# ShengkaiWu/IoU-aware-single-stage-object-detector

Hardware: AMD Instinct MI355X
Metric: images/sec at 1333x800, IoU-aware RetinaNet R-50-FPN (higher is better)
Workload: dtype fp32; 1 GPU; IoU-aware RetinaNet R-50-FPN fp32, batch 8 per GPU, 3x800x1344 (1333x800 padded to /32), random-init weights, whole inference path incl. NMS, device-to-host copy and bbox2result (the reference's simple_test: per-class arrays on the host; batch i's host part runs under batch i+1's device part, the last one inside the timed region); global_batch=8, parallelism=dp1, dets_per_image=100

## Files before the change

### include/iouaware.h

```cpp
#ifndef IOUAWARE_H
#define IOUAWARE_H

#include <stddef.h>
#include <stdint.h>

#ifdef __cplusplus
extern "C" {
#endif

#define IA_MAX_LEVELS 8
#define IA_MAX_ANCHORS 16
#define IA_MAX_NMS_PRE 4096
#define IA_MAX_CANDIDATES 8192
#define IA_MAX_PER_IMG 1024

#define IA_F32 0
#define IA_BF16 1
#define IA_F16 2
#define IA_F64 3

#define IA_LAYOUT_NCHW 0
#define IA_LAYOUT_NHWC 1

#define IA_CLS_SIGMOID 0
// ... 152 lines not shown
int ia_bn_fold_bwd(const float *dw_folded, const float *db_folded, const float *w, const float *gamma,
                   const float *mean, const float *inv_std, int cout, int K, float *dw,
                   float *dgamma, float *dbeta, void *stream);
int ia_relu_bwd_bias_grad(const float *dy, const float *y, int64_t rows, int n, float *g, float *db,
                          void *workspace, size_t workspace_bytes, void *stream);

int ia_linear_bias_act(const float *A, const float *W, const float *bias, const float *residual,
                       float *D, int64_t rows, int k, int n, int relu, void *workspace,
                       size_t workspace_bytes, void *stream);
int ia_linear_bias_act_bf16(const void *A, const void *W, const float *bias, const void *residual,
                            void *D, int64_t rows, int k, int n, int relu, void *workspace,
                            size_t workspace_bytes, void *stream);
int ia_batched_gemm(const float *A, const float *W, float *D, int batch, int64_t rows, int k, int n,
                    void *workspace, size_t workspace_bytes, void *stream);
int ia_batched_gemm_stream(const float *A, const float *W, float *D, int batch, int64_t rows, int k,
                           int n, void *stream);

size_t ia_im2col3x3_bytes(int B, int H, int W, int C, int stride, int dtype);
int ia_im2col3x3_nhwc(const void *x, void *col, int B, int H, int W, int C, int stride, int dtype,
                      void *stream);
int ia_conv1x1_strided(const void *x, const void *W_kn, const float *bias, const void *residual,
                       void *D, int B, int H, int W, int k, int n, int stride, int relu, int dtype,
                       void *workspace, size_t workspace_bytes, void *stream);
int ia_col2im3x3_nhwc(const void *dcol, void *dx, int B, int H, int W, int C, int stride, int dtype,
                      void *stream);

size_t ia_deform_im2col3x3_bytes(int B, int H, int W, int C, int stride, int pad, int dil);
int ia_deform_im2col3x3_nhwc(const float *x, const float *offset, int64_t offset_pix_stride,
                             const float *mask, int64_t mask_pix_stride, int mask_logits,
                             float *col, int B, int H, int W, int C, int stride, int pad,
                             int dil, int deformable_groups, void *stream);
int ia_deform_col2im3x3_nhwc(const float *dcol, const float *x, const float *offset,
                             int64_t offset_pix_stride, const float *mask,
                             int64_t mask_pix_stride, float *dx, float *d_offset, float *d_mask,
                             int B, int H, int W, int C, int stride, int pad, int dil,
                             int deformable_groups, void *stream);

int ia_gemm_tuning(int mode);

int ia_gemm_table_add(int64_t m, int64_t n, int64_t k, int flags, int batch, int dtype,
                      int solution_index);
int ia_gemm_table_clear(void);
int ia_gemm_table_dump(int64_t *rows7, int capacity);
int ia_gemm_table_stats(int64_t *hits_misses_stale);
int ia_gemm_library_version(void);

// ... 176 lines not shown

int ia_affine_relu_maxpool_nhwc(const float *x, const float *scale, const float *shift, int B, int H,
                                int W, int C, float *out, void *stream);
int ia_affine_relu_maxpool_nhwc_dt(const void *x, int dtype, const float *scale, const float *shift,
                                   int B, int H, int W, int C, void *out, void *stream);

int ia_upsample2x_add_nhwc(float *fine, const float *coarse, int B, int H, int W, int Hc, int Wc,
                           int C, void *stream);
int ia_upsample2x_add_nhwc_dt(void *fine, const void *coarse, int dtype, int B, int H, int W, int Hc,
                              int Wc, int C, void *stream);

int ia_stem_conv7x7s2(const float *x, const float *w_packed, float *y, int B, int H, int W,
                      void *stream);
int ia_stem_conv7x7s2_bf16(const void *x, const void *w_packed, void *y, int B, int H, int W,
                           void *stream);

int ia_conv1x1_stream(const float *x, const float *w, const float *bias, const float *residual,
                      float *y, int64_t rows, int k, int n, int relu, void *stream);
int ia_conv1x1_chain(const float *x, const float *w, const float *bias, const float *residual,
                     const float *w2, const float *bias2, float *y, float *h, int64_t rows, int k,
                     int n, int n2, void *stream);
int ia_conv1x1_wide(const float *x, const float *w, const float *bias, const float *residual,
                    float *y, int64_t rows, int k, int n, int relu, void *stream);

typedef struct ia_conv3x3_desc {
    int32_t num_levels, batch, groups;
    int32_t cin, cout;
    int32_t x_stride, y_stride;
    int32_t H[IA_MAX_LEVELS], W[IA_MAX_LEVELS];
    const void *x[2][IA_MAX_LEVELS];
    void *y[2][IA_MAX_LEVELS];
} ia_conv3x3_desc;
size_t ia_conv3x3_bf16_packed_bytes(int cin, int cout, int groups);
int ia_conv3x3_bf16_pack(const void *w, int cin, int cout, int groups, void *wp, void *stream);
int ia_conv3x3_bf16_levels(const ia_conv3x3_desc *d, const void *wp, const float *bias, int relu, void *stream);

size_t ia_conv3x3_bf16_wgrad_workspace_bytes(const ia_conv3x3_desc *d);
int ia_conv3x3_bf16_wgrad_plan(const ia_conv3x3_desc *d, int32_t *tiles, int32_t *slice_tiles, int32_t *slices);
int ia_conv3x3_bf16_wgrad_levels(const ia_conv3x3_desc *d, float *dw, void *workspace, size_t workspace_bytes,
                                 void *stream);
int ia_conv3x3_bf16_pack_f32(const float *w, int cin, int cout, int groups, int adjoint, void *wp, void *stream);
size_t ia_relu_bwd_bias_grad_bf16_workspace_bytes(int64_t rows, int n);
int ia_relu_bwd_bias_grad_bf16(const void *dy, int64_t dy_stride, const void *y, int64_t y_stride, int64_t rows,
                               int n, void *g, int64_t g_stride, float *db, void *workspace,
                               size_t workspace_bytes, void *stream);

// ... 155 lines not shown
```

### iou-aware-single-stage-object-detector_amd/csrc/build.py

```python
import os
import subprocess
import sys

HERE = os.path.dirname(os.path.abspath(__file__))
SOURCES = ['capi.hip', 'decode.hip', 'select.hip', 'nms.hip', 'loss.hip', 'elementwise.hip', 'assign.hip',
           'softnms.hip', 'preproc.hip', 'wino.hip', 'gemm.hip', 'lazynms.hip', 'headloss.hip', 'gconv.hip',
           'trainops.hip', 'bignms.hip', 'conv3x3_bf16.hip', 'conv3x3_bf16_bwd.hip', 'conv1x1_stream.hip', 'im2col.hip', 'nms64.hip', 'stem.hip',
           'groupnorm.hip', 'pointdecode.hip', 'pointloss.hip', 'gconv_bf16.hip', 'gconv_bwd.hip', 'deform.hip']
HEADERS = ['ia_math.hpp', 'ia_block.hpp', 'ia_internal.hpp', 'ia_loss.hpp', 'ia_headloss.hpp', 'ia_rowmax_dev.hpp', 'ia_gather_dev.hpp', 'ia_nms.hpp', 'ia_conv3.hpp', 'ia_wino.hpp', '../../include/iouaware.h']
OUT = os.path.join(HERE, 'libiouaware_hip.so')
FLAGS = ['--offload-arch=gfx950', '-O3', '-std=c++17', '-fPIC', '-ffp-contract=off',
         '-fhip-fp32-correctly-rounded-divide-sqrt', '-fno-gpu-rdc',
         '-Wall', '-Wno-unused-function']


def _hipcc():
    for c in (os.environ.get('HIPCC'), '/opt/rocm/bin/hipcc', 'hipcc'):
        if c and (os.path.isabs(c) and os.path.exists(c) or not os.path.isabs(c)):
            return c
    return 'hipcc'


def needs_build():
    if not os.path.exists(OUT):
        return True
    t = os.path.getmtime(OUT)
    deps = [os.path.join(HERE, f) for f in SOURCES + HEADERS] + [os.path.abspath(__file__)]
    return any(os.path.getmtime(d) > t for d in deps)


def build(force=False, verbose=False):
    if not force and not needs_build():
# ... 25 lines not shown
```

### iou-aware-single-stage-object-detector_amd/csrc/conv1x1_stream.hip

```cpp
#include <string.h>
#include <mutex>
#include <vector>
#include "ia_internal.hpp"

namespace ia {

typedef __attribute__((ext_vector_type(4))) float f32x4;

struct Conv1Args {
    const float *x, *w, *bias, *res;
    float *y;
    int64_t P;
    int32_t relu, tiles;
    int64_t xs, ws, ys;
};

constexpr int kC1Threads = 512;

template <int K, int N>
__global__ void __launch_bounds__(kC1Threads) __attribute__((amdgpu_waves_per_eu(4, 4))) k_conv1x1_stream(Conv1Args a)
{
    constexpr int NB = N / 16, J = K / 16, LDW = N + 4;
    __shared__ __attribute__((aligned(16))) float s_w[K * LDW];
    __shared__ __attribute__((aligned(16))) float s_bias[N];
    const int tid = threadIdx.x, lane = tid & 63;
    a.x += (size_t)blockIdx.y * a.xs; a.w += (size_t)blockIdx.y * a.ws; a.y += (size_t)blockIdx.y * a.ys;
// ... 117 lines not shown
                const float *wrow = wq + (16 * j + c) * LDW;
                constexpr int WB = NB > 8 ? 8 : NB;
#pragma unroll
                for (int n0 = 0; n0 < NB; n0 += WB) {
                    float wf[WB];
#pragma unroll
                    for (int nb = 0; nb < WB; ++nb) wf[nb] = wrow[16 * (n0 + nb)];
#pragma unroll
                    for (int nb = 0; nb < WB; ++nb)
                        acc[n0 + nb] = __builtin_amdgcn_mfma_f32_16x16x4f32(wf[nb], xb, acc[n0 + nb], 0, 0, 0);
                    if (n0 + WB < NB) __builtin_amdgcn_sched_barrier(0);
                }
                __builtin_amdgcn_sched_barrier(0);
            }
        if (p0 < a.P) {
            float *yr = a.y + p * a.ldn + n0 + 4 * q;
#pragma unroll
            for (int nb = 0; nb < NB; ++nb) {
                f32x4 v = acc[nb];
                if (a.relu) { v.x = v.x > 0.f ? v.x : 0.f; v.y = v.y > 0.f ? v.y : 0.f; v.z = v.z > 0.f ? v.z : 0.f; v.w = v.w > 0.f ? v.w : 0.f; }
                *reinterpret_cast<f32x4 *>(yr + 16 * nb) = v;
            }
        }
    }
}

struct ChainArgs {
    const float *x, *w, *bias, *res;
    const float *w2, *bias2;
    float *y, *h;
    int64_t P;
    int32_t tiles;
};

constexpr int kChainThreads = 1024;

template <int K, int N, int N2>
__global__ void __launch_bounds__(kChainThreads) __attribute__((amdgpu_waves_per_eu(4, 4))) k_conv1x1_chain(ChainArgs a)
{
    constexpr int NB = N / 16, J = K / 16, LDW = N + 4, NB2 = N2 / 16, LDW2 = N2 + 4;
    extern __shared__ __attribute__((aligned(16))) float s_dyn[];
    float *s_w = s_dyn, *s_w2 = s_w + K * LDW, *s_bias = s_w2 + N * LDW2, *s_bias2 = s_bias + N;
    const int tid = threadIdx.x, lane = tid & 63;
    for (int i = tid; i < K * (N / 4); i += kChainThreads) {
        const int k = i / (N / 4), n4 = i - k * (N / 4);
        *reinterpret_cast<float4 *>(s_w + k * LDW + 4 * n4) = *reinterpret_cast<const float4 *>(a.w + (size_t)k * N + 4 * n4);
// ... 186 lines not shown
    if (tiles > 2147483647LL) return IA_E_ARG;
    a.tiles = (int32_t)tiles;
    int64_t wgs = (tiles + 15) / 16;
    if (wgs > 128) wgs = 128;
    const size_t lds = sizeof(float) * (128 * (256 + 4) + 256);
    int dev = 0;
    if (hipGetDevice(&dev) != hipSuccess) return IA_E_ARG;
    {
        static std::mutex mu;
        static std::vector<char> done;
        std::lock_guard<std::mutex> lock(mu);
        if ((size_t)dev >= done.size()) done.resize((size_t)dev + 1, 0);
        if (!done[dev]) {
            hipError_t e = hipFuncSetAttribute(reinterpret_cast<const void *>(&ia::k_conv1x1_wide<128, 256>),
                                               hipFuncAttributeMaxDynamicSharedMemorySize, (int)lds);
            if (e != hipSuccess) return ia::hip_status(e);
            done[dev] = 1;
        }
    }
    hipLaunchKernelGGL((ia::k_conv1x1_wide<128, 256>), dim3((unsigned)wgs, 2), dim3(ia::kWideThreads), lds,
                       (hipStream_t)stream, a);
    return ia::hip_status(hipGetLastError());
}
```

### iou-aware-single-stage-object-detector_amd/csrc/im2col.hip

```cpp
#include "ia_internal.hpp"

namespace ia {

struct Im2colArgs {
    const uint4 *x;
    uint4 *col;
    int32_t B, H, W, Ho, Wo, stride;
    int32_t cv;
    int32_t lanes;
    int64_t runs;
};

__global__ __launch_bounds__(256) void k_im2col3x3(Im2colArgs a)
{
    const int lane = threadIdx.x & 63;
    const int sub = lane / a.lanes, l = lane - sub * a.lanes;
    const int per_wave = 64 / a.lanes;
    const int64_t wave = (int64_t)blockIdx.x * 4 + (threadIdx.x >> 6);
    for (int r = 0; r < 4; ++r) {
        const int64_t run = (wave * 4 + r) * per_wave + sub;
        if (run >= a.runs) return;
        const int64_t pix = run / 9;
        const int tap = (int)(run - pix * 9);
        const int dy = tap / 3, dx = tap - dy * 3;
        const int xo = (int)(pix % a.Wo);
        const int64_t t = pix / a.Wo;
        const int yo = (int)(t % a.Ho);
        const int b = (int)(t / a.Ho);
        const int yi = yo * a.stride + dy - 1, xi = xo * a.stride + dx - 1;
        const bool in = yi >= 0 && yi < a.H && xi >= 0 && xi < a.W;
        const uint4 *src = a.x + (((int64_t)b * a.H + (in ? yi : 0)) * a.W + (in ? xi : 0)) * a.cv;
        uint4 *dst = a.col + run * a.cv;
        for (int c = l; c < a.cv; c += a.lanes) {
            uint4 v = src[c];
            if (!in) v = make_uint4(0, 0, 0, 0);
            dst[c] = v;
        }
    }
}

struct Col2imArgs {
    const float4 *dcol;
    float4 *dx;
    int32_t H, W, Ho, Wo;
    int32_t cv;
    int32_t shift;
};

template <int S>
__global__ __launch_bounds__(256) void k_col2im3x3(Col2imArgs a)
{
    constexpr int NJ = (S + 2) / S;
    const int lane = threadIdx.x & 63;
    const int lanes = 1 << a.shift, sub = lane >> a.shift, l = lane & (lanes - 1);
    const int per_wave = 64 >> a.shift;
    const int xi = ((int)blockIdx.y * 4 + (int)(threadIdx.x >> 6)) * per_wave + sub;
    if (xi >= a.W) return;
    const int row = (int)blockIdx.x;
    const int b = row / a.H, yi = row - b * a.H;
    const int dy0 = (yi + 1) % S, dx0 = (xi + 1) % S;
    int64_t off[NJ * NJ];
    bool ok[NJ * NJ];
#pragma unroll
    for (int j = 0; j < NJ; ++j) {
        const int dy = dy0 + j * S, ny = yi + 1 - dy, yo = ny / S;
        const bool oky = dy < 3 && ny >= 0 && yo < a.Ho;
#pragma unroll
        for (int i = 0; i < NJ; ++i) {
            const int dx = dx0 + i * S, nx = xi + 1 - dx, xo = nx / S;
            const bool in = oky && dx < 3 && nx >= 0 && xo < a.Wo;
            ok[j * NJ + i] = in;
            off[j * NJ + i] = in ? ((((int64_t)b * a.Ho + yo) * a.Wo + xo) * 9 + (dy * 3 + dx)) * a.cv : 0;
        }
    }
    float4 *dst = a.dx + ((int64_t)row * a.W + xi) * a.cv;
    for (int c = l; c < a.cv; c += lanes) {
        float4 v[NJ * NJ];
#pragma unroll
        for (int t = 0; t < NJ * NJ; ++t) v[t] = a.dcol[off[t] + c];
        float4 acc = make_float4(0.0f, 0.0f, 0.0f, 0.0f);
#pragma unroll
        for (int t = 0; t < NJ * NJ; ++t)
            if (ok[t]) { acc.x += v[t].x; acc.y += v[t].y; acc.z += v[t].z; acc.w += v[t].w; }
        dst[c] = acc;
    }
}

}

extern "C" size_t ia_im2col3x3_bytes(int B, int H, int W, int C, int stride, int dtype)
{
    if (B < 1 || H < 1 || W < 1 || C < 1 || stride < 1 || (dtype != IA_F32 && dtype != IA_BF16)) return 0;
    const int64_t Ho = (H - 1) / stride + 1, Wo = (W - 1) / stride + 1;
// ... 2 lines not shown

extern "C" int ia_im2col3x3_nhwc(const void *x, void *col, int B, int H, int W, int C, int stride,
                                 int dtype, void *stream)
{
    if (!x || !col || B < 1 || H < 1 || W < 1 || C < 1 || stride < 1 || stride > 4) return IA_E_ARG;
    if (dtype != IA_F32 && dtype != IA_BF16) return IA_E_ARG;
    const int esz = dtype == IA_F32 ? 4 : 2;
    if ((C * esz) % 16) return IA_E_ARG;
    if (((uintptr_t)x | (uintptr_t)col) & 15) return IA_E_ARG;
    ia::Im2colArgs a;
    a.x = (const uint4 *)x; a.col = (uint4 *)col;
    a.B = B; a.H = H; a.W = W; a.stride = stride;
    a.Ho = (H - 1) / stride + 1; a.Wo = (W - 1) / stride + 1;
    a.cv = C * esz / 16;
    int lanes = 64;
    while (lanes > a.cv) lanes >>= 1;
    a.lanes = lanes < 1 ? 1 : lanes;
    a.runs = (int64_t)B * a.Ho * a.Wo * 9;
    const int64_t per_block = 16LL * (64 / a.lanes);
    const int64_t blocks = (a.runs + per_block - 1) / per_block;
    if (blocks > 2147483647LL) return IA_E_ARG;
    hipLaunchKernelGGL(ia::k_im2col3x3, dim3((unsigned)blocks), dim3(256), 0, (hipStream_t)stream, a);
    return ia::hip_status(hipGetLastError());
}

extern "C" int ia_col2im3x3_nhwc(const void *dcol, void *dx, int B, int H, int W, int C, int stride,
                                 int dtype, void *stream)
{
    if (!dcol || !dx || B < 1 || H < 1 || W < 1 || C < 1 || stride < 1 || stride > 4) return IA_E_ARG;
    if (dtype != IA_F32 || C % 4) return IA_E_ARG;
    if (((uintptr_t)dcol | (uintptr_t)dx) & 15) return IA_E_ARG;
    ia::Col2imArgs a;
    a.dcol = (const float4 *)dcol; a.dx = (float4 *)dx;
    a.H = H; a.W = W;
    a.Ho = (H - 1) / stride + 1; a.Wo = (W - 1) / stride + 1;
    a.cv = C / 4;
    a.shift = 0;
    while (a.shift < 6 && (2 << a.shift) <= a.cv) ++a.shift;
    const int64_t rows = (int64_t)B * H;
    const int per_block = 4 * (64 >> a.shift);
    const int chunks = (W + per_block - 1) / per_block;
    if (rows > 2147483647LL || chunks > 65535) return IA_E_ARG;
    const dim3 grid((unsigned)rows, (unsigned)chunks), block(256);
    hipStream_t s = (hipStream_t)stream;
    switch (stride) {
    case 1: hipLaunchKernelGGL(ia::k_col2im3x3<1>, grid, block, 0, s, a); break;
// ... 7 lines not shown
```

### iou-aware-single-stage-object-detector_amd/iouaware/_lib.py

```python
import ctypes as C
import os

IA_MAX_LEVELS = 8
IA_MAX_ANCHORS = 16
IA_MAX_NMS_PRE = 4096
IA_MAX_CANDIDATES = 8192
IA_MAX_PER_IMG = 1024
IA_F32, IA_BF16, IA_F16, IA_F64 = 0, 1, 2, 3
IA_LAYOUT_NCHW, IA_LAYOUT_NHWC = 0, 1
IA_CLS_SIGMOID, IA_CLS_SOFTMAX = 0, 1
IA_CLS_SIGMOID_NOIOU, IA_CLS_SOFTMAX_NOIOU = 2, 3
IA_LOSS_SLOTS = 64
IA_MAX_TARGET_BATCH = 16
IA_GN_CHUNK = 256

_CSRC = os.path.join(os.path.dirname(os.path.abspath(__file__)), '..', 'csrc')
SO_PATH = os.path.abspath(os.path.join(_CSRC, 'libiouaware_hip.so'))


class HeadGeom(C.Structure):
    _fields_ = [('num_levels', C.c_int32), ('num_anchors', C.c_int32),
                ('num_classes', C.c_int32), ('nms_pre', C.c_int32),
                ('H', C.c_int32 * IA_MAX_LEVELS), ('W', C.c_int32 * IA_MAX_LEVELS),
                ('stride', C.c_int32 * IA_MAX_LEVELS),
# ... 130 lines not shown
                                     _vp, _vp]),
    'ia_wino_grad_output_transform': (_i, [C.POINTER(WinoGeom), C.POINTER(C.c_void_p), _i, _vp, _vp]),
    'ia_wino_weight_transform': (_i, [_vp, _i, _i, C.c_int64, C.c_int64, C.c_int64, C.c_int64, _i,
                                      C.POINTER(C.c_double), _vp, _vp]),
    'ia_wino_weight_grad': (_i, [_vp, _i, _i, C.POINTER(C.c_double), _vp, C.c_int64, C.c_int64,
                                 C.c_int64, C.c_int64, _vp]),
    'ia_bn_fold_fwd': (_i, [_vp, _vp, _vp, _vp, _vp, _i, _i, _vp, _vp, _vp]),
    'ia_bn_fold_bwd': (_i, [_vp, _vp, _vp, _vp, _vp, _vp, _i, _i, _vp, _vp, _vp, _vp]),
    'ia_relu_bwd_bias_grad_workspace_bytes': (C.c_size_t, [C.c_int64, _i]),
    'ia_relu_bwd_bias_grad': (_i, [_vp, _vp, C.c_int64, _i, _vp, _vp, _vp, C.c_size_t, _vp]),
    'ia_wino_output_transform': (_i, [C.POINTER(WinoGeom), _vp, _i, _i, _vp, _i, _i,
                                      C.POINTER(WinoSeg), _vp]),
    'ia_wino_mid_transform': (_i, [C.POINTER(WinoGeom), _vp, _i, _i, _vp, _i, _vp, _i, _vp]),
    'ia_wino_in_gemm': (_i, [C.POINTER(WinoGeom), C.POINTER(C.c_void_p), _i, _vp, _vp, _i, _vp, _vp, _vp]),
    'ia_linear_bias_act': (_i, [_vp, _vp, _vp, _vp, _vp, _i64, _i, _i, _i, _vp, _sz, _vp]),
    'ia_linear_bias_act_bf16': (_i, [_vp, _vp, _vp, _vp, _vp, _i64, _i, _i, _i, _vp, _sz, _vp]),
    'ia_batched_gemm': (_i, [_vp, _vp, _vp, _i, _i64, _i, _i, _vp, _sz, _vp]),
    'ia_batched_gemm_stream': (_i, [_vp, _vp, _vp, _i, _i64, _i, _i, _vp]),
    'ia_linear_bias_act_wt': (_i, [_vp, _vp, _vp, _vp, _vp, _i64, _i, _i, _i, _vp, _sz, _vp]),
    'ia_gemm_tuning': (_i, [_i]),
    'ia_im2col3x3_bytes': (_sz, [_i, _i, _i, _i, _i, _i]),
    'ia_im2col3x3_nhwc': (_i, [_vp, _vp, _i, _i, _i, _i, _i, _i, _vp]),
    'ia_col2im3x3_nhwc': (_i, [_vp, _vp, _i, _i, _i, _i, _i, _i, _vp]),
    'ia_deform_im2col3x3_bytes': (_sz, [_i, _i, _i, _i, _i, _i, _i]),
    'ia_deform_im2col3x3_nhwc': (_i, [_vp, _vp, _i64, _vp, _i64, _i, _vp, _i, _i, _i, _i, _i, _i, _i, _i, _vp]),
    'ia_deform_col2im3x3_nhwc': (_i, [_vp, _vp, _vp, _i64, _vp, _i64, _vp, _vp, _vp, _i, _i, _i, _i, _i, _i,
                                      _i, _i, _vp]),
    'ia_conv1x1_strided': (_i, [_vp, _vp, _vp, _vp, _vp, _i, _i, _i, _i, _i, _i, _i, _i, _vp, _sz, _vp]),
    'ia_gemm_table_add': (_i, [_i64, _i64, _i64, _i, _i, _i, _i]),
    'ia_gemm_table_clear': (_i, []),
    'ia_gemm_table_dump': (_i, [_vp, _i]),
    'ia_gemm_table_stats': (_i, [_vp]),
    'ia_gemm_library_version': (_i, []),
    'ia_gemm_tn': (_i, [_vp, _vp, _vp, _i, _i64, _i, _i, _vp, _sz, _vp]),
    'ia_focal_loss_fwd': (_i, [_vp, _i, _vp, _vp, _i, _i, _i, _i, _f, _f, _vp, _vp]),
    'ia_focal_loss_bwd': (_i, [_vp, _i, _vp, _vp, _i, _i, _i, _i, _f, _f, _f, _vp, _vp, _vp]),
    'ia_smooth_l1_fwd': (_i, [_vp, _i, _vp, _vp, _i, _i, _i, _f, _vp, _vp]),
    'ia_smooth_l1_bwd': (_i, [_vp, _i, _vp, _vp, _i, _i, _i, _f, _f, _vp, _vp, _vp]),
    'ia_balanced_l1_fwd': (_i, [_vp, _i, _vp, _vp, _i, _i, _i, _f, _f, _f, _vp, _vp]),
    'ia_balanced_l1_bwd': (_i, [_vp, _i, _vp, _vp, _i, _i, _i, _f, _f, _f, _f, _vp, _vp, _vp]),
    'ia_focal_loss_balanced_fwd': (_i, [_vp, _i, _vp, _vp, _vp, _i, _i, _i, _i, _f, _f, _f, _vp, _vp]),
    'ia_focal_loss_balanced_bwd': (_i, [_vp, _i, _vp, _vp, _vp, _i, _i, _i, _i, _f, _f, _f, _vp, _f,
                                        _vp, _vp, _vp]),
    'ia_smooth_l1_balanced_fwd': (_i, [_vp, _i, _vp, _vp, _vp, _i, _i, _i, _f, _f, _vp, _vp]),
    'ia_smooth_l1_balanced_bwd': (_i, [_vp, _i, _vp, _vp, _vp, _i, _i, _i, _f, _f, _f, _vp, _vp,
                                       _vp]),
# ... 25 lines not shown
                                       C.POINTER(HeadLossCfg), C.POINTER(BoxLossCfg), _vp, _vp, _P,
                                       C.POINTER(LevelPixStrides), _vp]),
    'ia_grouped_conv3x3_pack': (_i, [_vp, _vp, _i, _i, _vp]),
    'ia_grouped_conv3x3_nhwc': (_i, [_vp, _vp, _vp, _vp, _i, _i, _i, _i, _i, _i, _i, _vp]),
    'ia_grouped_conv3x3_packed_bytes_bf16': (C.c_size_t, [_i, _i]),
    'ia_grouped_conv3x3_pack_dev': (_i, [_vp, _vp, _i, _i, _i, _vp, _vp]),
    'ia_grouped_conv3x3_bwd_data_nhwc': (_i, [_vp, _vp, _vp, _i, _i, _i, _i, _i, _i, _vp]),
    'ia_grouped_conv3x3_bwd_weight_workspace_bytes': (C.c_size_t, [_i, _i, _i, _i, _i, _i]),
    'ia_grouped_conv3x3_bwd_weight_nhwc': (_i, [_vp, _vp, _vp, _vp, C.c_size_t, _i, _i, _i, _i, _i, _i, _vp]),
    'ia_grouped_conv3x3_pack_bf16': (_i, [_vp, _vp, _i, _i, _vp]),
    'ia_grouped_conv3x3_bf16_nhwc': (_i, [_vp, _vp, _vp, _vp, _i, _i, _i, _i, _i, _i, _i, _vp]),
    'ia_sigmoid_focal_loss_fwd': (_i, [_vp, _vp, _i, _i, _f, _f, _vp, _vp]),
    'ia_sigmoid_focal_loss_bwd': (_i, [_vp, _vp, _vp, _i, _i, _f, _f, _vp, _vp]),
    'ia_sigmoid_focal_loss_fwd_dt': (_i, [_vp, _i, _vp, _i, _i, _f, _f, _vp, _vp]),
    'ia_sigmoid_focal_loss_bwd_dt': (_i, [_vp, _i, _vp, _vp, _i, _i, _f, _f, _vp, _vp]),
    'ia_channel_affine_act': (_i, [_vp, _i, _vp, _vp, _vp, _vp, _vp, _i, _i, _i, _i64, _vp]),
    'ia_channel_affine_act_nhwc': (_i, [_vp, _i, _vp, _vp, _vp, _vp, _vp, _i, _i64, _i, _vp]),
    'ia_nhwc_to_nchw': (_i, [_vp, _vp, _i, _i, _i, _i64, _vp]),
    'ia_upsample2x_add_nhwc': (_i, [_vp, _vp, _i, _i, _i, _i, _i, _i, _vp]),
    'ia_conv1x1_stream': (_i, [_vp, _vp, _vp, _vp, _vp, C.c_int64, _i, _i, _i, _vp]),
    'ia_stem_conv7x7s2': (_i, [_vp, _vp, _vp, _i, _i, _i, _vp]),
    'ia_stem_conv7x7s2_bf16': (_i, [_vp, _vp, _vp, _i, _i, _i, _vp]),
    'ia_conv1x1_wide': (_i, [_vp, _vp, _vp, _vp, _vp, C.c_int64, _i, _i, _i, _vp]),
    'ia_conv1x1_chain': (_i, [_vp, _vp, _vp, _vp, _vp, _vp, _vp, _vp, _i64, _i, _i, _i, _vp]),
    'ia_conv3x3_bf16_packed_bytes': (C.c_size_t, [_i, _i, _i]),
    'ia_conv3x3_bf16_pack': (_i, [_vp, _i, _i, _i, _vp, _vp]),
    'ia_conv3x3_bf16_levels': (_i, [_vp, _vp, _vp, _i, _vp]),
    'ia_conv3x3_bf16_wgrad_workspace_bytes': (C.c_size_t, [_vp]),
    'ia_conv3x3_bf16_wgrad_plan': (_i, [_vp, C.POINTER(C.c_int32), C.POINTER(C.c_int32), C.POINTER(C.c_int32)]),
    'ia_conv3x3_bf16_wgrad_levels': (_i, [_vp, _vp, _vp, C.c_size_t, _vp]),
    'ia_conv3x3_bf16_pack_f32': (_i, [_vp, _i, _i, _i, _i, _vp, _vp]),
    'ia_relu_bwd_bias_grad_bf16_workspace_bytes': (C.c_size_t, [C.c_int64, _i]),
    'ia_relu_bwd_bias_grad_bf16': (_i, [_vp, C.c_int64, _vp, C.c_int64, C.c_int64, _i, _vp, C.c_int64, _vp,
                                        _vp, C.c_size_t, _vp]),
    'ia_upsample2x_add_nhwc_dt': (_i, [_vp, _vp, _i, _i, _i, _i, _i, _i, _i, _vp]),
    'ia_affine_relu_maxpool_nhwc_dt': (_i, [_vp, _i, _vp, _vp, _i, _i, _i, _i, _vp, _vp]),
    'ia_affine_relu_maxpool_nhwc': (_i, [_vp, _vp, _vp, _i, _i, _i, _i, _vp, _vp]),
    'ia_groupnorm_workspace_bytes': (_sz, [_WG, _i, _i]),
    'ia_groupnorm_stats': (_i, [_WG, C.POINTER(C.c_void_p), _i, _i, _vp, _sz, _vp]),
    'ia_groupnorm_apply': (_i, [_WG, C.POINTER(C.c_void_p), _i, _i, _vp, _vp, _f, _i, _vp, _sz, _vp]),
    'ia_groupnorm_workspace_bytes_dt': (_sz, [_WG, _i, _i, _i]),
    'ia_groupnorm_stats_dt': (_i, [_WG, C.POINTER(C.c_void_p), _i, _i, _i, _vp, _sz, _vp]),
    'ia_groupnorm_apply_dt': (_i, [_WG, C.POINTER(C.c_void_p), _i, _i, _i, _vp, _vp, _f, _i, _vp, _sz,
                                   _vp]),
    'ia_groupnorm_saved_bytes': (_sz, [_WG, _i, _i]),
    'ia_groupnorm_apply_to': (_i, [_WG, C.POINTER(C.c_void_p), C.POINTER(C.c_void_p), _i, _i, _vp, _vp, _f,
# ... 80 lines not shown
```

### iou-aware-single-stage-object-detector_amd/iouaware/fuse.py

```python
import types

import torch
import torch.nn.functional as F
from torch.nn.modules.batchnorm import _BatchNorm

from . import ops, train_fuse
from .backbones import BasicBlock, Bottleneck, ResNet
from .deform_conv import _DeformBase, _one
from .layers import ConvModule, Scale
from .winograd import plain_3x3

_VEC = {torch.float32: 4, torch.bfloat16: 8}


def _fold_bn(bn):
    if not isinstance(bn, _BatchNorm):
        raise TypeError('only BatchNorm can be folded, got %s' % type(bn).__name__)
    with torch.no_grad():
        var, mean = bn.running_var.float(), bn.running_mean.float()
        g = bn.weight.float() if bn.weight is not None else torch.ones_like(var)
        b = bn.bias.float() if bn.bias is not None else torch.zeros_like(var)
        scale = g / torch.sqrt(var + bn.eps)
        shift = b - mean * scale
    return scale.contiguous(), shift.contiguous()
# ... 85 lines not shown
        return ops.channel_affine_act_(self._conv2(out), f['s2'], f['b2'], relu=True)
    co, c2 = self.conv2_offset, self.conv2
    if 'off_im2col' in f:
        om = ops.conv3x3_im2col(out, f['off_im2col'], f['off_b'], stride=co.stride[0])
    elif 'off_wino' in f and f['off_wino'].usable(out):
        om = f['off_wino'](out)
    else:
        om = co(out).contiguous(memory_format=torch.channels_last)
    n = 18 * self.deformable_groups
    return ops.deform_conv3x3(out, om[:, :n], om[:, n:] if self.with_modulated_dcn else None, f['dcn2'],
                              f['b2'], _one(c2.stride, 'stride'), _one(c2.padding, 'padding'),
                              _one(c2.dilation, 'dilation'), self.deformable_groups, relu=True,
                              mask_logits=True)


def _bottleneck_run(self, x, h1=None, nxt=None):
    if not _fast(self, x):
        if _train(self) and train_fuse.bottleneck_usable(self, x):
            return train_fuse.bottleneck_forward(self, x), None
        return type(self).forward(self, x), None
    f = self._ia_fused
    lt = 'w1' in f and x.dtype in (torch.float32, torch.bfloat16) \
        and x.is_contiguous(memory_format=torch.channels_last)
    if h1 is not None:
        w, out, pre = f, h1, None
    elif lt:
        w = _weights_for(f, x.dtype)
        out, pre = ops.linear_bias_act(x, w['w1'], f['b1'], relu=True), None
    else:
        out, pre = self.conv1(x), (f['s1'], f['b1'], True)
    gw = f.get('gconv2')
    wino = f.get('wino2')
    if getattr(self, 'with_dcn', False):
        if pre is not None:
            out = ops.channel_affine_act_(out, f['s1'], f['b1'], relu=True)
        out = _dcn_conv2(self, f, out)
    elif gw is not None and out.dtype == torch.float32 \
            and out.is_contiguous(memory_format=torch.channels_last):
        if pre is not None:
            out = ops.channel_affine_act_(out, f['s1'], f['b1'], relu=True)
        out = ops.grouped_conv3x3(out, gw, f['b2'], self.conv2.groups, self.conv2.stride[0],
                                  relu=True)
    elif gw is not None and out.dtype == torch.bfloat16 and self.conv2.in_channels % 32 == 0 \
            and out.is_contiguous(memory_format=torch.channels_last) and self._ia_gconv_bf16:
        if pre is not None:
            out = ops.channel_affine_act_(out, f['s1'], f['b1'], relu=True)
        wp = f.get('_gconv2_bf16')
        if wp is None:
            wp = f['_gconv2_bf16'] = ops.pack_grouped_weight_bf16(self.conv2.weight, f['s2'])
        out = ops.grouped_conv3x3_bf16(out, wp, f['b2'], self.conv2.groups, self.conv2.stride[0],
                                       relu=True)
    elif wino is not None and wino.usable(out):
        out = wino(out, pre=pre)
    elif pre is None and 'c3' in f and out.dtype == torch.bfloat16 \
            and out.is_contiguous(memory_format=torch.channels_last):
        wp = f.get('_c3_packed')
# ... 479 lines not shown
```

### iou-aware-single-stage-object-detector_amd/iouaware/ops.py

```python
import ctypes as C
import os

import numpy as np
import torch

from . import _lib
from ._lib import HeadGeom, LevelPtrs, IA_F32, IA_BF16


_raw_stream = getattr(torch._C, '_cuda_getCurrentRawStream', None)


def stream_id():
    if _raw_stream is not None:
        return _raw_stream(torch.cuda.current_device())
    return torch.cuda.current_stream().cuda_stream


def _stream():
    return C.c_void_p(stream_id())


def _ptr(t):
    return C.c_void_p(t.data_ptr()) if t is not None else C.c_void_p(0)
# ... 844 lines not shown

_CHAIN_SHAPE = (64, 256, 64)
CHAIN_1X1 = True


def chain_usable(x, k, n, n2):
    return CHAIN_1X1 and STREAM_1X1 and x.dtype == torch.float32 and (k, n, n2) == _CHAIN_SHAPE \
        and x.shape[0] * x.shape[2] * x.shape[3] >= 65536


_col_cache = {}


def _col_buffer(device, nbytes):
    key = (device.index, stream_id())
    buf = _col_cache.get(key)
    if buf is None or buf.numel() < nbytes:
        buf = None
        _col_cache.pop(key, None)
        buf = _col_cache[key] = torch.empty(int(nbytes), dtype=torch.uint8, device=device)
    return buf


def conv3x3_im2col(x, w_kn, bias=None, stride=2, relu=False):
    _require_gpu(x, 'x')
    B, Cc, H, W = x.shape
    n = int(w_kn.shape[1])
    if x.dtype not in (torch.float32, torch.bfloat16) or not x.is_contiguous(memory_format=torch.channels_last):
        raise TypeError('conv3x3_im2col needs a channels-last fp32 / bf16 activation')
    if tuple(w_kn.shape) != (9 * Cc, n) or not w_kn.is_contiguous() or w_kn.dtype != x.dtype:
        raise ValueError('weight must be a contiguous (9 * C, Cout) matrix of the activation dtype')
    if bias is not None and bias.dtype != torch.float32:
        raise TypeError('bias must be fp32')
    dt = _dtype_code(x)
    L = _lib.lib()
    nbytes = L.ia_im2col3x3_bytes(B, H, W, Cc, int(stride), dt)
    if nbytes == 0 or (Cc * x.element_size()) % 16:
        raise ValueError('conv3x3_im2col: C * sizeof(dtype) must be a multiple of 16')
    col = _col_buffer(x.device, nbytes)
    Ho, Wo = (H - 1) // stride + 1, (W - 1) // stride + 1
    _lib.check(L.ia_im2col3x3_nhwc(_ptr(x), _ptr(col), B, H, W, Cc, int(stride), dt, _stream()),
               'ia_im2col3x3_nhwc')
    out = torch.empty((B, n, Ho, Wo), dtype=x.dtype, device=x.device, memory_format=torch.channels_last)
    _ensure_gemm_table()
    ws = _workspace(x.device, _LT_WS_BYTES)
    fn = L.ia_linear_bias_act if x.dtype == torch.float32 else L.ia_linear_bias_act_bf16
    _lib.check(fn(_ptr(col), _ptr(w_kn), _ptr(bias), None, _ptr(out), B * Ho * Wo, 9 * Cc, n,
                  int(bool(relu)), _ptr(ws), _LT_WS_BYTES, _stream()), 'ia_linear_bias_act (im2col)')
    return out


def im2col3x3(x, stride):
    _require_gpu(x, 'x')
    B, Cc, H, W = x.shape
    if x.dtype != torch.float32 or not x.is_contiguous(memory_format=torch.channels_last):
        raise TypeError('im2col3x3 needs a channels-last fp32 activation')
    stride = int(stride)
    if Cc % 4 or not 1 <= stride <= 4:
        raise ValueError('im2col3x3: C a multiple of 4, stride 1..4')
    rows = B * ((H - 1) // stride + 1) * ((W - 1) // stride + 1)
    nbytes = rows * 9 * Cc * 4
    col = _col_buffer(x.device, nbytes)
    _lib.check(_lib.lib().ia_im2col3x3_nhwc(_ptr(x), _ptr(col), B, H, W, Cc, stride, IA_F32, _stream()),
               'ia_im2col3x3_nhwc')
    return col[:nbytes].view(torch.float32).view(rows, 9 * Cc)


def conv3x3_dcol(g, w_kn):
    _require_gpu(g, 'g')
    B, n, Ho, Wo = g.shape
    if g.dtype != torch.float32 or not g.is_contiguous(memory_format=torch.channels_last):
        raise TypeError('conv3x3_dcol needs a channels-last fp32 gradient')
    if w_kn.dim() != 2 or w_kn.shape[1] != n or w_kn.shape[0] % 9 or not w_kn.is_contiguous() \
            or w_kn.dtype != torch.float32:
        raise ValueError('weight must be the contiguous fp32 (9 * C, Cout) matrix of the forward')
    rows, k9 = B * Ho * Wo, int(w_kn.shape[0])
    nbytes = rows * k9 * 4
    col = _col_buffer(g.device, nbytes)
    _ensure_gemm_table()
    ws = _workspace(g.device, _LT_WS_BYTES)
    _lib.check(_lib.lib().ia_linear_bias_act_wt(_ptr(g), _ptr(w_kn), None, None, _ptr(col), rows, n, k9, 0,
                                                _ptr(ws), _LT_WS_BYTES, _stream()),
               'ia_linear_bias_act_wt (dcol)')
    return col[:nbytes].view(torch.float32).view(rows, k9)


def col2im3x3(dcol, B, H, W, C, stride):
    _require_gpu(dcol, 'dcol')
# ... 1092 lines not shown
```

Baseline: 417.1 img/s.

## Fuse 1x1 conv into stride-2 im2col scatter and add scatter im2col

```diff
diff --git a/include/iouaware.h b/include/iouaware.h
--- a/include/iouaware.h
+++ b/include/iouaware.h
@@ -198,6 +198,8 @@
 int ia_conv1x1_strided(const void *x, const void *W_kn, const float *bias, const void *residual,
                        void *D, int B, int H, int W, int k, int n, int stride, int relu, int dtype,
                        void *workspace, size_t workspace_bytes, void *stream);
+int ia_im2col3x3_scatter_nhwc(const void *x, void *col, int B, int H, int W, int C, int stride,
+                              int dtype, void *stream);
 int ia_col2im3x3_nhwc(const void *dcol, void *dx, int B, int H, int W, int C, int stride, int dtype,
                       void *stream);
 
@@ -420,6 +422,8 @@
                      int n, int n2, void *stream);
 int ia_conv1x1_wide(const float *x, const float *w, const float *bias, const float *residual,
                     float *y, int64_t rows, int k, int n, int relu, void *stream);
+int ia_conv1x1_im2col(const float *x, const float *w, const float *bias, float *out, int B, int H,
+                      int W, int k, int n, int stride, int dtype, int relu, int col, void *stream);
 
 typedef struct ia_conv3x3_desc {
     int32_t num_levels, batch, groups;
diff --git a/iou-aware-single-stage-object-detector_amd/csrc/build.py b/iou-aware-single-stage-object-detector_amd/csrc/build.py
--- a/iou-aware-single-stage-object-detector_amd/csrc/build.py
+++ b/iou-aware-single-stage-object-detector_amd/csrc/build.py
@@ -7,7 +7,7 @@
            'softnms.hip', 'preproc.hip', 'wino.hip', 'gemm.hip', 'lazynms.hip', 'headloss.hip', 'gconv.hip',
            'trainops.hip', 'bignms.hip', 'conv3x3_bf16.hip', 'conv3x3_bf16_bwd.hip', 'conv1x1_stream.hip', 'im2col.hip', 'nms64.hip', 'stem.hip',
            'groupnorm.hip', 'pointdecode.hip', 'pointloss.hip', 'gconv_bf16.hip', 'gconv_bwd.hip', 'deform.hip']
-HEADERS = ['ia_math.hpp', 'ia_block.hpp', 'ia_internal.hpp', 'ia_loss.hpp', 'ia_headloss.hpp', 'ia_rowmax_dev.hpp', 'ia_gather_dev.hpp', 'ia_nms.hpp', 'ia_conv3.hpp', 'ia_wino.hpp', '../../include/iouaware.h']
+HEADERS = ['ia_math.hpp', 'ia_block.hpp', 'ia_internal.hpp', 'ia_loss.hpp', 'ia_headloss.hpp', 'ia_rowmax_dev.hpp', 'ia_gather_dev.hpp', 'ia_nms.hpp', 'ia_conv3.hpp', 'ia_wino.hpp', 'ia_colmap.hpp', '../../include/iouaware.h']
 OUT = os.path.join(HERE, 'libiouaware_hip.so')
 FLAGS = ['--offload-arch=gfx950', '-O3', '-std=c++17', '-fPIC', '-ffp-contract=off',
          '-fhip-fp32-correctly-rounded-divide-sqrt', '-fno-gpu-rdc',
diff --git a/iou-aware-single-stage-object-detector_amd/csrc/conv1x1_stream.hip b/iou-aware-single-stage-object-detector_amd/csrc/conv1x1_stream.hip
--- a/iou-aware-single-stage-object-detector_amd/csrc/conv1x1_stream.hip
+++ b/iou-aware-single-stage-object-detector_amd/csrc/conv1x1_stream.hip
@@ -2,6 +2,7 @@
 #include <mutex>
 #include <vector>
 #include "ia_internal.hpp"
+#include "ia_colmap.hpp"
 
 namespace ia {
 
@@ -165,6 +166,88 @@
                 *reinterpret_cast<f32x4 *>(yr + 16 * nb) = v;
             }
         }
+    }
+}
+
+struct ColArgs {
+    const float *x, *w, *bias;
+    float *y;
+    int32_t P, tiles, relu, col;
+    int32_t H, W, Ho, Wo;
+};
+
+template <int K, int NT>
+__global__ void __launch_bounds__(kWideThreads) __attribute__((amdgpu_waves_per_eu(4, 4))) k_conv1x1_col(ColArgs a)
+{
+    constexpr int NB = NT / 16, J = K / 16, LDW = NT + 4;
+    extern __shared__ __attribute__((aligned(16))) float s_dyn[];
+    float *s_w = s_dyn, *s_bias = s_w + K * LDW;
+    const int tid = threadIdx.x, lane = tid & 63;
+    for (int i = tid; i < K * (NT / 4); i += kWideThreads) {
+        const int k = i / (NT / 4), n4 = i - k * (NT / 4);
+        *reinterpret_cast<float4 *>(s_w + k * LDW + 4 * n4) = *reinterpret_cast<const float4 *>(a.w + (size_t)k * NT + 4 * n4);
+    }
+    for (int i = tid; i < NT; i += kWideThreads) s_bias[i] = a.bias ? a.bias[i] : 0.0f;
+    __syncthreads();
+
+    const int p_in = lane & 15, q = lane >> 4;
+    const int wave = (tid >> 6) * gridDim.x + blockIdx.x, nwaves = gridDim.x * (kWideThreads / 64);
+    const float *wq = s_w + (4 * q) * LDW + p_in;
+    for (int tile = wave; tile < a.tiles; tile += nwaves) {
+        const int p0 = tile * 16 + p_in, plast = a.P - 1;
+        const int p = p0 < plast ? p0 : plast;
+        const float *xr = a.x + ((int64_t)p * K + 4 * q);
+        f32x4 xv[J];
+#pragma unroll
+        for (int j = 0; j < J; ++j) xv[j] = *reinterpret_cast<const f32x4 *>(xr + 16 * j);
+        f32x4 acc[NB];
+#pragma unroll
+        for (int nb = 0; nb < NB; ++nb) acc[nb] = f32x4{0.0f, 0.0f, 0.0f, 0.0f};
+#pragma unroll
+        for (int nb = 0; nb < NB; ++nb) {
+            const f32x4 bz = *reinterpret_cast<const f32x4 *>(s_bias + 16 * nb + 4 * q);
+            acc[nb] += bz;
+        }
+#pragma unroll
+        for (int j = 0; j < J; ++j)
+#pragma unroll
+            for (int c = 0; c < 4; ++c) {
+                const float xb = xv[j][c];
+                const float *wrow = wq + (16 * j + c) * LDW;
+                float wf[NB];
+#pragma unroll
+                for (int nb = 0; nb < NB; ++nb) wf[nb] = wrow[16 * nb];
+#pragma unroll
+                for (int nb = 0; nb < NB; ++nb)
+                    acc[nb] = __builtin_amdgcn_mfma_f32_16x16x4f32(wf[nb], xb, acc[nb], 0, 0, 0);
+                __builtin_amdgcn_sched_barrier(0);
+            }
+        if (a.relu) {
+#pragma unroll
+            for (int nb = 0; nb < NB; ++nb) {
+                f32x4 v = acc[nb];
+                v.x = v.x > 0.f ? v.x : 0.f; v.y = v.y > 0.f ? v.y : 0.f; v.z = v.z > 0.f ? v.z : 0.f; v.w = v.w > 0.f ? v.w : 0.f;
+                acc[nb] = v;
+            }
+        }
+        if (p0 > plast) continue;
+        if (!a.col) {
+            float *yr = a.y + ((int64_t)p * NT + 4 * q);
+#pragma unroll
+            for (int nb = 0; nb < NB; ++nb) *reinterpret_cast<f32x4 *>(yr + 16 * nb) = acc[nb];
+            continue;
+        }
+        const int xi = p % a.W, t = p / a.W, yi = t % a.H, b = t / a.H;
+        col_runs_of_pixel<2>(b, yi, xi, a.H, a.W, a.Ho, a.Wo, [&](int64_t run, bool real) {
+            float *yr = a.y + (run * NT + 4 * q);
+            if (real) {
+#pragma unroll
+                for (int nb = 0; nb < NB; ++nb) *reinterpret_cast<f32x4 *>(yr + 16 * nb) = acc[nb];
+            } else {
+#pragma unroll
+                for (int nb = 0; nb < NB; ++nb) *reinterpret_cast<f32x4 *>(yr + 16 * nb) = f32x4{0.0f, 0.0f, 0.0f, 0.0f};
+            }
+        });
     }
 }
 
@@ -397,3 +480,37 @@
                        (hipStream_t)stream, a);
     return ia::hip_status(hipGetLastError());
 }
+
+extern "C" int ia_conv1x1_im2col(const float *x, const float *w, const float *bias, float *out, int B, int H,
+                                 int W, int k, int n, int stride, int dtype, int relu, int col, void *stream)
+{
+    if (!x || !w || !out || B < 1 || H < 1 || W < 1) return IA_E_ARG;
+    if (dtype != IA_F32 || k != 256 || n != 128 || stride != 2) return IA_E_ARG;
+    if (((uintptr_t)x & 15u) || ((uintptr_t)w & 15u) || ((uintptr_t)out & 15u)) return IA_E_ARG;
+    const int64_t rows = (int64_t)B * H * W;
+    if (rows > 2147483647LL - 16) return IA_E_ARG;
+    ia::ColArgs a;
+    a.x = x; a.w = w; a.bias = bias; a.y = out; a.P = (int32_t)rows; a.relu = relu ? 1 : 0; a.col = col ? 1 : 0;
+    a.H = H; a.W = W; a.Ho = (H - 1) / 2 + 1; a.Wo = (W - 1) / 2 + 1;
+    a.tiles = (int32_t)((rows + 15) / 16);
+    int64_t wgs = (a.tiles + 15) / 16;
+    if (wgs > 256) wgs = 256;
+    const size_t lds = sizeof(float) * (256 * (128 + 4) + 128);
+    int dev = 0;
+    if (hipGetDevice(&dev) != hipSuccess) return IA_E_ARG;
+    {
+        static std::mutex mu;
+        static std::vector<char> done;
+        std::lock_guard<std::mutex> lock(mu);
+        if ((size_t)dev >= done.size()) done.resize((size_t)dev + 1, 0);
+        if (!done[dev]) {
+            hipError_t e = hipFuncSetAttribute(reinterpret_cast<const void *>(&ia::k_conv1x1_col<256, 128>),
+                                               hipFuncAttributeMaxDynamicSharedMemorySize, (int)lds);
+            if (e != hipSuccess) return ia::hip_status(e);
+            done[dev] = 1;
+        }
+    }
+    hipLaunchKernelGGL((ia::k_conv1x1_col<256, 128>), dim3((unsigned)wgs), dim3(ia::kWideThreads), lds,
+                       (hipStream_t)stream, a);
+    return ia::hip_status(hipGetLastError());
+}
diff --git a/iou-aware-single-stage-object-detector_amd/csrc/ia_colmap.hpp b/iou-aware-single-stage-object-detector_amd/csrc/ia_colmap.hpp
--- /dev/null
+++ b/iou-aware-single-stage-object-detector_amd/csrc/ia_colmap.hpp
@@ -0,0 +1,38 @@
+#pragma once
+#include <stdint.h>
+#include <hip/hip_runtime.h>
+
+namespace ia {
+
+template <int S>
+__device__ __forceinline__ bool col_axis_tap(int i, int j, int no, int &d, int &o)
+{
+    d = (i + 1) % S + j * S;
+    const int n = i + 1 - d;
+    o = n / S;
+    return d < 3 && n >= 0 && o < no;
+}
+
+template <int S, class F>
+__device__ __forceinline__ void col_runs_of_pixel(int b, int yi, int xi, int H, int W, int Ho, int Wo, F &&f)
+{
+    constexpr int NJ = (S + 2) / S;
+    for (int vy = -1; vy <= 1; ++vy) {
+        if ((vy < 0 && yi != 0) || (vy > 0 && yi != H - 1)) continue;
+        for (int jy = 0; jy < NJ; ++jy) {
+            int dy, yo;
+            if (!col_axis_tap<S>(yi + vy, jy, Ho, dy, yo)) continue;
+            const int64_t row = ((int64_t)b * Ho + yo) * Wo;
+            for (int vx = -1; vx <= 1; ++vx) {
+                if ((vx < 0 && xi != 0) || (vx > 0 && xi != W - 1)) continue;
+                for (int jx = 0; jx < NJ; ++jx) {
+                    int dx, xo;
+                    if (!col_axis_tap<S>(xi + vx, jx, Wo, dx, xo)) continue;
+                    f((row + xo) * 9 + (dy * 3 + dx), vy == 0 && vx == 0);
+                }
+            }
+        }
+    }
+}
+
+}
diff --git a/iou-aware-single-stage-object-detector_amd/csrc/im2col.hip b/iou-aware-single-stage-object-detector_amd/csrc/im2col.hip
--- a/iou-aware-single-stage-object-detector_amd/csrc/im2col.hip
+++ b/iou-aware-single-stage-object-detector_amd/csrc/im2col.hip
@@ -1,4 +1,5 @@
 #include "ia_internal.hpp"
+#include "ia_colmap.hpp"
 
 namespace ia {
 
@@ -39,6 +40,48 @@
     }
 }
 
+struct Im2colScatterArgs {
+    const uint4 *x;
+    uint4 *col;
+    int32_t H, W, Ho, Wo;
+    int32_t cv;
+    int32_t shift;
+};
+
+__global__ __launch_bounds__(256) void k_im2col3x3_scatter(Im2colScatterArgs a)
+{
+    const int lane = threadIdx.x & 63;
+    const int lanes = 1 << a.shift, sub = lane >> a.shift, l = lane & (lanes - 1);
+    const int per_wave = 64 >> a.shift;
+    const int xi = ((int)blockIdx.y * 4 + (int)(threadIdx.x >> 6)) * per_wave + sub;
+    if (xi >= a.W) return;
+    const int row = (int)blockIdx.x;
+    const int b = row / a.H, yi = row - b * a.H;
+    const uint4 *src = a.x + ((int64_t)row * a.W + xi) * a.cv;
+    for (int c = l; c < a.cv; c += lanes) {
+        const uint4 v = src[c];
+        col_runs_of_pixel<2>(b, yi, xi, a.H, a.W, a.Ho, a.Wo, [&](int64_t run, bool real) {
+            a.col[run * a.cv + c] = real ? v : make_uint4(0, 0, 0, 0);
+        });
+    }
+}
+
+static int im2col_scatter(const void *x, void *col, int B, int H, int W, int cv, hipStream_t stream)
+{
+    Im2colScatterArgs a;
+    a.x = (const uint4 *)x; a.col = (uint4 *)col;
+    a.H = H; a.W = W; a.Ho = (H - 1) / 2 + 1; a.Wo = (W - 1) / 2 + 1;
+    a.cv = cv;
+    a.shift = 0;
+    while (a.shift < 6 && (2 << a.shift) <= a.cv) ++a.shift;
+    const int64_t rows = (int64_t)B * H;
+    const int per_block = 4 * (64 >> a.shift);
+    const int chunks = (W + per_block - 1) / per_block;
+    if (rows > 2147483647LL || chunks > 65535) return IA_E_ARG;
+    hipLaunchKernelGGL(k_im2col3x3_scatter, dim3((unsigned)rows, (unsigned)chunks), dim3(256), 0, stream, a);
+    return hip_status(hipGetLastError());
+}
+
 struct Col2imArgs {
     const float4 *dcol;
     float4 *dx;
@@ -58,17 +101,15 @@
     if (xi >= a.W) return;
     const int row = (int)blockIdx.x;
     const int b = row / a.H, yi = row - b * a.H;
-    const int dy0 = (yi + 1) % S, dx0 = (xi + 1) % S;
     int64_t off[NJ * NJ];
     bool ok[NJ * NJ];
 #pragma unroll
     for (int j = 0; j < NJ; ++j) {
-        const int dy = dy0 + j * S, ny = yi + 1 - dy, yo = ny / S;
-        const bool oky = dy < 3 && ny >= 0 && yo < a.Ho;
+        int dy, yo, dx, xo;
+        const bool oky = col_axis_tap<S>(yi, j, a.Ho, dy, yo);
 #pragma unroll
         for (int i = 0; i < NJ; ++i) {
-            const int dx = dx0 + i * S, nx = xi + 1 - dx, xo = nx / S;
-            const bool in = oky && dx < 3 && nx >= 0 && xo < a.Wo;
+            const bool in = col_axis_tap<S>(xi, i, a.Wo, dx, xo) && oky;
             ok[j * NJ + i] = in;
             off[j * NJ + i] = in ? ((((int64_t)b * a.Ho + yo) * a.Wo + xo) * 9 + (dy * 3 + dx)) * a.cv : 0;
         }
@@ -117,6 +158,17 @@
     if (blocks > 2147483647LL) return IA_E_ARG;
     hipLaunchKernelGGL(ia::k_im2col3x3, dim3((unsigned)blocks), dim3(256), 0, (hipStream_t)stream, a);
     return ia::hip_status(hipGetLastError());
+}
+
+extern "C" int ia_im2col3x3_scatter_nhwc(const void *x, void *col, int B, int H, int W, int C, int stride,
+                                         int dtype, void *stream)
+{
+    if (!x || !col || B < 1 || H < 1 || W < 1 || C < 1 || stride != 2) return IA_E_ARG;
+    if (dtype != IA_F32 && dtype != IA_BF16) return IA_E_ARG;
+    const int esz = dtype == IA_F32 ? 4 : 2;
+    if ((C * esz) % 16) return IA_E_ARG;
+    if (((uintptr_t)x | (uintptr_t)col) & 15) return IA_E_ARG;
+    return ia::im2col_scatter(x, col, B, H, W, C * esz / 16, (hipStream_t)stream);
 }
 
 extern "C" int ia_col2im3x3_nhwc(const void *dcol, void *dx, int B, int H, int W, int C, int stride,
diff --git a/iou-aware-single-stage-object-detector_amd/iouaware/_lib.py b/iou-aware-single-stage-object-detector_amd/iouaware/_lib.py
--- a/iou-aware-single-stage-object-detector_amd/iouaware/_lib.py
+++ b/iou-aware-single-stage-object-detector_amd/iouaware/_lib.py
@@ -176,6 +176,7 @@
     'ia_im2col3x3_bytes': (_sz, [_i, _i, _i, _i, _i, _i]),
     'ia_im2col3x3_nhwc': (_i, [_vp, _vp, _i, _i, _i, _i, _i, _i, _vp]),
     'ia_col2im3x3_nhwc': (_i, [_vp, _vp, _i, _i, _i, _i, _i, _i, _vp]),
+    'ia_im2col3x3_scatter_nhwc': (_i, [_vp, _vp, _i, _i, _i, _i, _i, _i, _vp]),
     'ia_deform_im2col3x3_bytes': (_sz, [_i, _i, _i, _i, _i, _i, _i]),
     'ia_deform_im2col3x3_nhwc': (_i, [_vp, _vp, _i64, _vp, _i64, _i, _vp, _i, _i, _i, _i, _i, _i, _i, _i, _vp]),
     'ia_deform_col2im3x3_nhwc': (_i, [_vp, _vp, _vp, _i64, _vp, _i64, _vp, _vp, _vp, _i, _i, _i, _i, _i, _i,
@@ -247,6 +248,7 @@
     'ia_stem_conv7x7s2': (_i, [_vp, _vp, _vp, _i, _i, _i, _vp]),
     'ia_stem_conv7x7s2_bf16': (_i, [_vp, _vp, _vp, _i, _i, _i, _vp]),
     'ia_conv1x1_wide': (_i, [_vp, _vp, _vp, _vp, _vp, C.c_int64, _i, _i, _i, _vp]),
+    'ia_conv1x1_im2col': (_i, [_vp, _vp, _vp, _vp, _i, _i, _i, _i, _i, _i, _i, _i, _i, _vp]),
     'ia_conv1x1_chain': (_i, [_vp, _vp, _vp, _vp, _vp, _vp, _vp, _vp, _i64, _i, _i, _i, _vp]),
     'ia_conv3x3_bf16_packed_bytes': (C.c_size_t, [_i, _i, _i]),
     'ia_conv3x3_bf16_pack': (_i, [_vp, _i, _i, _i, _vp, _vp]),
diff --git a/iou-aware-single-stage-object-detector_amd/iouaware/fuse.py b/iou-aware-single-stage-object-detector_amd/iouaware/fuse.py
--- a/iou-aware-single-stage-object-detector_amd/iouaware/fuse.py
+++ b/iou-aware-single-stage-object-detector_amd/iouaware/fuse.py
@@ -131,16 +131,24 @@
     f = self._ia_fused
     lt = 'w1' in f and x.dtype in (torch.float32, torch.bfloat16) \
         and x.is_contiguous(memory_format=torch.channels_last)
+    gw = f.get('gconv2')
+    wino = f.get('wino2')
+    col = False
     if h1 is not None:
         w, out, pre = f, h1, None
+    elif lt and 'im2col2' in f and gw is None and wino is None and not getattr(self, 'with_dcn', False) \
+            and ops.col_1x1_usable(x, f['w1'], self.conv2.stride[0]):
+        w, pre, col = f, None, True
+        out = ops.conv1x1_im2col_conv3x3(x, f['w1'], f['b1'], f['im2col2'], f['b2'],
+                                         stride=self.conv2.stride[0], relu=True)
     elif lt:
         w = _weights_for(f, x.dtype)
         out, pre = ops.linear_bias_act(x, w['w1'], f['b1'], relu=True), None
     else:
         out, pre = self.conv1(x), (f['s1'], f['b1'], True)
-    gw = f.get('gconv2')
-    wino = f.get('wino2')
-    if getattr(self, 'with_dcn', False):
+    if col:
+        pass
+    elif getattr(self, 'with_dcn', False):
         if pre is not None:
             out = ops.channel_affine_act_(out, f['s1'], f['b1'], relu=True)
         out = _dcn_conv2(self, f, out)
diff --git a/iou-aware-single-stage-object-detector_amd/iouaware/ops.py b/iou-aware-single-stage-object-detector_amd/iouaware/ops.py
--- a/iou-aware-single-stage-object-detector_amd/iouaware/ops.py
+++ b/iou-aware-single-stage-object-detector_amd/iouaware/ops.py
@@ -890,6 +890,9 @@
     return buf
 
 
+SCATTER_IM2COL = True
+
+
 def conv3x3_im2col(x, w_kn, bias=None, stride=2, relu=False):
     _require_gpu(x, 'x')
     B, Cc, H, W = x.shape
@@ -907,8 +910,10 @@
         raise ValueError('conv3x3_im2col: C * sizeof(dtype) must be a multiple of 16')
     col = _col_buffer(x.device, nbytes)
     Ho, Wo = (H - 1) // stride + 1, (W - 1) // stride + 1
-    _lib.check(L.ia_im2col3x3_nhwc(_ptr(x), _ptr(col), B, H, W, Cc, int(stride), dt, _stream()),
-               'ia_im2col3x3_nhwc')
+    scatter = SCATTER_IM2COL and int(stride) == 2 and x.dtype == torch.float32 and Cc >= 512
+    fn = L.ia_im2col3x3_scatter_nhwc if scatter else L.ia_im2col3x3_nhwc
+    _lib.check(fn(_ptr(x), _ptr(col), B, H, W, Cc, int(stride), dt, _stream()),
+               'ia_im2col3x3_scatter_nhwc' if scatter else 'ia_im2col3x3_nhwc')
     out = torch.empty((B, n, Ho, Wo), dtype=x.dtype, device=x.device, memory_format=torch.channels_last)
     _ensure_gemm_table()
     ws = _workspace(x.device, _LT_WS_BYTES)
@@ -932,6 +937,74 @@
     _lib.check(_lib.lib().ia_im2col3x3_nhwc(_ptr(x), _ptr(col), B, H, W, Cc, stride, IA_F32, _stream()),
                'ia_im2col3x3_nhwc')
     return col[:nbytes].view(torch.float32).view(rows, 9 * Cc)
+
+
+def im2col3x3_scatter(x, out=None):
+    _require_gpu(x, 'x')
+    B, Cc, H, W = x.shape
+    if x.dtype not in (torch.float32, torch.bfloat16) or not x.is_contiguous(memory_format=torch.channels_last):
+        raise TypeError('im2col3x3_scatter needs a channels-last fp32 / bf16 activation')
+    rows = B * ((H - 1) // 2 + 1) * ((W - 1) // 2 + 1)
+    if out is None:
+        out = torch.empty(rows * 9 * Cc, dtype=x.dtype, device=x.device)
+    if out.dtype != x.dtype or out.numel() != rows * 9 * Cc or not out.is_contiguous():
+        raise ValueError('im2col3x3_scatter: out must be a contiguous (rows * 9 * C) buffer of the dtype')
+    _lib.check(_lib.lib().ia_im2col3x3_scatter_nhwc(_ptr(x), _ptr(out), B, H, W, Cc, 2, _dtype_code(x),
+                                                    _stream()), 'ia_im2col3x3_scatter_nhwc')
+    return out.view(rows, 9 * Cc)
+
+
+_COL_SHAPE = (256, 128)
+COL_1X1 = True
+COL_1X1_MIN_PIXELS = 65536
+
+
+def conv1x1_im2col(x, w_kn, bias=None, relu=True, col=True, out=None):
+    _require_gpu(x, 'x')
+    B, k, H, W = x.shape
+    if x.dtype != torch.float32 or not x.is_contiguous(memory_format=torch.channels_last) \
+            or tuple(w_kn.shape) != _COL_SHAPE or k != _COL_SHAPE[0] or w_kn.dtype != torch.float32 \
+            or not w_kn.is_contiguous():
+        raise TypeError('conv1x1_im2col: fp32 channels-last input, (k, n) = %s' % (_COL_SHAPE,))
+    n = _COL_SHAPE[1]
+    if bias is not None and (bias.dtype != torch.float32 or bias.numel() != n or not bias.is_contiguous()):
+        raise TypeError('conv1x1_im2col: bias is a contiguous fp32 vector of the output width')
+    shape = (B * ((H - 1) // 2 + 1) * ((W - 1) // 2 + 1), 9 * n) if col else (B * H * W, n)
+    if out is None:
+        out = torch.empty(shape[0] * shape[1], dtype=torch.float32, device=x.device)
+    if out.dtype != torch.float32 or out.numel() != shape[0] * shape[1] or not out.is_contiguous():
+        raise ValueError('conv1x1_im2col: out must be a contiguous fp32 buffer of %d elements' % (shape[0] * shape[1]))
+    _lib.check(_lib.lib().ia_conv1x1_im2col(_ptr(x), _ptr(w_kn), _ptr(bias), _ptr(out), B, H, W, k, n, 2, IA_F32,
+                                            int(bool(relu)), int(bool(col)), _stream()), 'ia_conv1x1_im2col')
+    return out.view(shape)
+
+
+def col_1x1_usable(x, w1_kn, stride):
+    return COL_1X1 and x.dtype == torch.float32 and tuple(w1_kn.shape) == _COL_SHAPE and int(stride) == 2 \
+        and x.shape[0] * x.shape[2] * x.shape[3] >= COL_1X1_MIN_PIXELS
+
+
+def conv1x1_im2col_conv3x3(x, w1_kn, b1, w2_kn, b2, stride=2, relu=True):
+    _require_gpu(x, 'x')
+    B, k, H, W = x.shape
+    n1, n = int(w1_kn.shape[1]), int(w2_kn.shape[1])
+    if int(stride) != 2:
+        raise ValueError('conv1x1_im2col_conv3x3: stride 2')
+    if tuple(w2_kn.shape) != (9 * n1, n) or not w2_kn.is_contiguous() or w2_kn.dtype != torch.float32:
+        raise ValueError('weight must be a contiguous fp32 (9 * C, Cout) matrix')
+    if b2 is not None and b2.dtype != torch.float32:
+        raise TypeError('bias must be fp32')
+    Ho, Wo = (H - 1) // 2 + 1, (W - 1) // 2 + 1
+    nbytes = B * Ho * Wo * 9 * n1 * 4
+    col = _col_buffer(x.device, nbytes)
+    conv1x1_im2col(x, w1_kn, b1, relu=True, col=True, out=col[:nbytes].view(torch.float32))
+    out = torch.empty((B, n, Ho, Wo), dtype=torch.float32, device=x.device, memory_format=torch.channels_last)
+    _ensure_gemm_table()
+    ws = _workspace(x.device, _LT_WS_BYTES)
+    _lib.check(_lib.lib().ia_linear_bias_act(_ptr(col), _ptr(w2_kn), _ptr(b2), None, _ptr(out), B * Ho * Wo,
+                                             9 * n1, n, int(bool(relu)), _ptr(ws), _LT_WS_BYTES, _stream()),
+               'ia_linear_bias_act (im2col)')
+    return out
 
 
 def conv3x3_dcol(g, w_kn):
```

Measured after the change: 419.6 img/s (median of 6 runs). No clear change (+0.6%).
